# rasmusab/bayes.js

Hardware: AMD Instinct MI355X
Metric: posterior draws/sec (= param-updates/sec) (higher is better)
Workload: dtype f64

## Files before the change

### bayes.js_amd/csrc/amwg_kernel.h

```cpp
#pragma once
#if !defined(__HIPCC_RTC__)
#include <hip/hip_runtime.h>
#endif

#include "amwg_div.h"
#include "amwg_ld.h"
#include "amwg_philox.h"
#include "amwg_types.h"

namespace amwg {

struct LdsLayout {
  uint32_t data, state, pls, cnt, tot, cc, adapt, pl, idx, perm, total, stride, logpls, bc, xw;
};
__host__ __device__ inline LdsLayout lds_layout(size_t data_bytes, int P, int CPB, int max_top, int n_named, bool multi = false) {
  LdsLayout L;
  uint32_t o = 0;
  L.stride = (uint32_t)P | 1u;
  L.data = o;  o += (uint32_t)((data_bytes + 15) & ~(size_t)15);
  L.state = o; o += L.stride * CPB * 8;
  L.pls = o;   o += L.stride * CPB * 8;
  L.cnt = o;   o += L.stride * CPB * 8;
  L.tot = o;   o += (L.stride * CPB * 4 + 15) & ~15u;
  L.cc = o;    o += (uint32_t)P * sizeof(CompConst);
  L.adapt = o; o += ((uint32_t)P + 7) & ~7u;
  L.pl = o;    o += (uint32_t)n_named * 20u;
  o = (o + 15) & ~15u;
  L.idx = o;   o += (max_top > 1) ? (((uint32_t)max_top * CPB * (max_top > kByteTop ? 2u : 1u) + 15) & ~15u) : 0;
  L.perm = o;  o += (n_named > kPackedNamed) ? (((uint32_t)n_named * CPB * 2u + 15) & ~15u) : 0;
  L.logpls = o; o += multi ? L.stride * CPB * 8 : 0;
  L.bc = o;     o += multi ? ((L.stride * CPB * 4 + 15) & ~15u) : 0;
  L.xw = o;     o += multi ? 2u * 16u * 8u : 0;
  L.total = (o + 15) & ~15u;
  return L;
}

template <class Model, bool FAST, int G, int U = Model::kUnroll>
__device__ __forceinline__ double pass_over_data(const typename Model::Pass &ps, int n_obs, int sub, double acc) {
  const int n_full = n_obs / G, rem = n_obs % G;
  int k = 0;
  for (; k + U <= n_full; k += U) {
    double t[U];
#pragma unroll
    for (int u = 0; u < U; ++u) t[u] = Model::template term<FAST>(ps, (k + u) * G + sub);
#pragma unroll
    for (int u = 0; u < U; ++u) acc += t[u];
  }
  for (; k < n_full; ++k) acc += Model::template term<FAST>(ps, k * G + sub);
  if (sub < rem) acc += Model::template term<FAST>(ps, n_full * G + sub);
  return acc;
}

struct CrossWave {
  double *buf;
  int parity;
};

template <class...> using void_of = void;

template <class M, class = void> struct BinaryOf { static constexpr bool value = true; };
template <class M> struct BinaryOf<M, void_of<decltype(M::kHasBinary)>> { static constexpr bool value = M::kHasBinary; };

template <class M, class = void> struct TracksState { static constexpr bool value = false; };
template <class M> struct TracksState<M, void_of<decltype(M::kTracksState)>> { static constexpr bool value = M::kTracksState; };

template <class M, class = void> struct LaneReuseOf { static constexpr bool value = false; };
template <class M> struct LaneReuseOf<M, void_of<decltype(M::kLaneReuse)>> { static constexpr bool value = M::kLaneReuse; };

template <class M, class = void> struct CertifiedOf { static constexpr bool value = false; static constexpr int lanes = 0; };
template <class M> struct CertifiedOf<M, void_of<decltype(M::kCertified)>> { static constexpr bool value = M::kCertified; static constexpr int lanes = M::kCertifiedLanes; };
template <class M, int G, class = void> struct CertifiedAt { static constexpr bool value = false; };
template <class M, int G> struct CertifiedAt<M, G, void_of<decltype(M::kCertified)>> { static constexpr bool value = M::kCertified && M::kCertifiedLanes == G; };

template <class M, class = void> struct CertNeedsRows { static constexpr bool value = false; };
template <class M> struct CertNeedsRows<M, void_of<decltype(M::kCertifiedNeedsRows)>> { static constexpr bool value = M::kCertifiedNeedsRows; };

template <class M, class = void> struct RefOrderOf { static constexpr bool value = false; };
template <class M> struct RefOrderOf<M, void_of<decltype(M::kReferenceOrder)>> { static constexpr bool value = M::kReferenceOrder; };

template <class M, class = void> struct OwnPassOf { static constexpr bool value = false; };
template <class M> struct OwnPassOf<M, void_of<decltype(M::kOwnPass)>> { static constexpr bool value = M::kOwnPass; };

struct NoCache {};
template <class M, class = void> struct CacheOf { using type = NoCache; static __device__ __forceinline__ type init() { return type{}; } };
template <class M> struct CacheOf<M, void_of<typename M::Cache>> { using type = typename M::Cache; static __device__ __forceinline__ type init() { return M::cache_init(); } };

template <int OFF, bool EXACT = false>
__device__ __forceinline__ double xor_partner(double v) {
#if defined(__HIP_DEVICE_COMPILE__)
  int lo = (int)(uint32_t)f64_bits(v), hi = (int)(uint32_t)(f64_bits(v) >> 32);
  if constexpr (OFF == 1) {
    lo = __builtin_amdgcn_mov_dpp(lo, 0xB1, 0xF, 0xF, true); hi = __builtin_amdgcn_mov_dpp(hi, 0xB1, 0xF, 0xF, true);
  } else if constexpr (OFF == 2) {
    lo = __builtin_amdgcn_mov_dpp(lo, 0x4E, 0xF, 0xF, true); hi = __builtin_amdgcn_mov_dpp(hi, 0x4E, 0xF, 0xF, true);
  } else if constexpr (OFF == 4) {
    lo = __builtin_amdgcn_mov_dpp(lo, 0x141, 0xF, 0xF, true); hi = __builtin_amdgcn_mov_dpp(hi, 0x141, 0xF, 0xF, true);
    if constexpr (EXACT) {
      lo = __builtin_amdgcn_mov_dpp(lo, 0x1B, 0xF, 0xF, true); hi = __builtin_amdgcn_mov_dpp(hi, 0x1B, 0xF, 0xF, true);
    }
  } else if constexpr (OFF == 8) {
    lo = __builtin_amdgcn_mov_dpp(lo, 0x140, 0xF, 0xF, true); hi = __builtin_amdgcn_mov_dpp(hi, 0x140, 0xF, 0xF, true);
    if constexpr (EXACT) {
      lo = __builtin_amdgcn_mov_dpp(lo, 0x141, 0xF, 0xF, true); hi = __builtin_amdgcn_mov_dpp(hi, 0x141, 0xF, 0xF, true);
    }
  } else if constexpr (OFF == 16) {
    lo = __builtin_amdgcn_ds_swizzle(lo, 0x401F); hi = __builtin_amdgcn_ds_swizzle(hi, 0x401F);
  } else {
    return __shfl_xor(v, OFF, 64);
  }
  return bits_f64(((uint64_t)(uint32_t)hi << 32) | (uint64_t)(uint32_t)lo);
#else
  return v;
#endif
}
template <int OFF, bool EXACT = false>
__device__ __forceinline__ double xor_sum(double acc) {
#if defined(__HIP_DEVICE_COMPILE__)
  if constexpr (OFF == 16 || OFF == 32) {
    const uint32_t lo = (uint32_t)f64_bits(acc), hi = (uint32_t)(f64_bits(acc) >> 32);
    if constexpr (OFF == 32) {
      const auto l = __builtin_amdgcn_permlane32_swap(lo, lo, false, false), h = __builtin_amdgcn_permlane32_swap(hi, hi, false, false);
      return bits_f64(((uint64_t)h[0] << 32) | (uint64_t)l[0]) + bits_f64(((uint64_t)h[1] << 32) | (uint64_t)l[1]);
    } else {
      const auto l = __builtin_amdgcn_permlane16_swap(lo, lo, false, false), h = __builtin_amdgcn_permlane16_swap(hi, hi, false, false);
      return bits_f64(((uint64_t)h[0] << 32) | (uint64_t)l[0]) + bits_f64(((uint64_t)h[1] << 32) | (uint64_t)l[1]);
    }
  } else {
    return acc + xor_partner<OFF, EXACT>(acc);
  }
#else
  return acc;
#endif
}
template <int OFF, int LIMIT>
__device__ __forceinline__ double butterfly(double acc) {
  if constexpr (OFF < LIMIT) { acc = xor_sum<OFF>(acc); return butterfly<OFF * 2, LIMIT>(acc); }
  else return acc;
}

#ifndef AMWG_STEPPER_PRIORITY
#define AMWG_STEPPER_PRIORITY 2
#endif
constexpr int kStepperPriority = AMWG_STEPPER_PRIORITY;
__device__ __forceinline__ void wave_priority(int p) {
#if defined(__HIP_DEVICE_COMPILE__)
  if (kStepperPriority > 0) { if (p == 0) __builtin_amdgcn_s_setprio(0); else __builtin_amdgcn_s_setprio(kStepperPriority); }
#endif
}

__device__ __forceinline__ int fresh_uniform(int v) {
#if defined(__HIP_DEVICE_COMPILE__)
#if !defined(AMWG_X_NOFRESH)
  v = __builtin_amdgcn_readfirstlane(v);
  asm volatile("" : "+s"(v));
#endif
#endif
  return v;
}

template <class Model, int G, int U = 8>
__device__ __forceinline__ double log_post(const StateView &S, const StepArgs &a0, const unsigned char *smem, int sub, CrossWave &xw,
                                           typename CacheOf<Model>::type &cache) {
  struct { const ModelConsts &mc; DataRef d; } a{a0.mc, a0.d};
  a.d.n_obs = fresh_uniform(a0.d.n_obs);
  a.d.G = fresh_uniform(a0.d.G);
  double acc;
  if constexpr (Model::kUser) {
    wave_priority(0);
    bool summed = false;
    if constexpr (LaneReuseOf<Model>::value && G == 64) {
      if (a0.d.pad > 0) { acc = Model::template rows_eval<U>(cache, S, a.d, smem, sub, a0.d.pad, (int)(threadIdx.x >> 6)); summed = true; }
    }
    if (!summed) acc = Model::template eval<G, false>(S, a.d, smem, sub, nullptr);
  } else {
    if constexpr (TracksState<Model>::value) Model::template load<G>(cache, S, a.mc, a.d, smem, sub);
    const typename Model::Pass ps = Model::template begin<G>(S, a.mc, a.d, smem, cache);
    const double prior = Model::prior(S, a.mc, a.d, cache);
    acc = (sub == 0) ? prior : 0.0;
    if constexpr (Model::kSplitPrior) acc = Model::template prior_split<G>(S, a.mc, a.d, sub, acc, cache);
    wave_priority(0);
    bool summed = false;
    if constexpr (LaneReuseOf<Model>::value && G == 64) {
      if (ps.rows) { acc = Model::template lane_sum_rows<U>(cache, ps, acc, a.d.n_obs, a.d.G, sub, smem, a0.d.pad, (int)(threadIdx.x >> 6)); summed = true; }
    }
    if (summed) {
    } else if constexpr (Model::kHasFast) {
      if (ps.fast) acc = Model::template pass_fast<G, U>(ps, a.d.n_obs, sub, acc);
      else acc = Model::template pass_slow<G>(ps, a.d.n_obs, sub, acc);
    } else if constexpr (Model::kOneLanePass && G == 1) {
      acc = Model::pass_one_lane(ps, a.d.n_obs, acc);
    } else if constexpr (OwnPassOf<Model>::value) {
      acc = Model::template pass<G>(ps, a.d.n_obs, sub, acc);
    } else {
      acc = pass_over_data<Model, false, G>(ps, a.d.n_obs, sub, acc);
    }
    if constexpr (Model::kOneLanePass) {
      if (ps.has_invalid) acc = acc + (-kInf);
    }
  }
  wave_priority(kStepperPriority);
  acc = butterfly<1, (G < 64 ? G : 64)>(acc);
  if constexpr (G > 64) {
    constexpr int WV = G / 64;
    double *slot = xw.buf + xw.parity * 16;
    xw.parity ^= 1;
    const int wave = sub >> 6;
    if ((sub & 63) == 0) slot[wave] = acc;
    __syncthreads();
    double t[WV];
#pragma unroll
    for (int w = 0; w < WV; ++w) t[w] = slot[w];
#pragma unroll
    for (int off = 1; off < WV; off <<= 1) {
      double u[WV];
#pragma unroll
      for (int w = 0; w < WV; ++w) u[w] = t[w] + t[w ^ off];
#pragma unroll
      for (int w = 0; w < WV; ++w) t[w] = u[w];
    }
    acc = t[0];
  }
  return acc;
}

template <int G>
struct CoopStream {
  static constexpr int L = G < 64 ? G : 64;
  static constexpr int kLanesPerChain = G;
  uint32_t k0, k1, c2, c3;
  uint64_t b0;
  uint32_t pos;
  double u0, u1;
  int lane_in_chain, base_lane;
  static __device__ __attribute__((noinline)) Philox4 block(uint64_t b, uint32_t c2, uint32_t c3, uint32_t k0, uint32_t k1) {
    return philox4x32_10((uint32_t)b, (uint32_t)(b >> 32), c2, c3, k0, k1);
  }
  __device__ __forceinline__ void set_block(const Philox4 &w) { u0 = u53(w.w0, w.w1); u1 = u53(w.w2, w.w3); }
  __device__ __forceinline__ void fill() { set_block(block(b0 + (uint64_t)lane_in_chain, c2, c3, k0, k1)); }
  __device__ __forceinline__ void init(uint64_t seed, uint64_t chain, uint64_t consumed, int tid) {
    k0 = (uint32_t)seed; k1 = (uint32_t)(seed >> 32);
    c2 = (uint32_t)chain; c3 = (uint32_t)(chain >> 32);
    lane_in_chain = tid & (L - 1);
    base_lane = (tid & 63) & ~(L - 1);
    b0 = consumed >> 1;
    pos = (uint32_t)(consumed & 1u);
    fill();
  }
  __device__ __forceinline__ uint64_t consumed() const { return 2 * b0 + (uint64_t)pos; }
  __device__ __forceinline__ double next() {
    if constexpr (L == 64) {
      uint32_t p = (uint32_t)__builtin_amdgcn_readfirstlane((int)pos);
      if (p >= 128u) { b0 += 64ull; p = 0u; fill(); }
      const double mine = (p & 1u) ? u1 : u0;
      const int src = (int)(p >> 1);
      const uint32_t hi = (uint32_t)__builtin_amdgcn_readlane((int)(f64_bits(mine) >> 32), src);
      const uint32_t lo = (uint32_t)__builtin_amdgcn_readlane((int)(uint32_t)f64_bits(mine), src);
      pos = p + 1u;
      return bits_f64(((uint64_t)hi << 32) | (uint64_t)lo);
    } else {
      if (pos >= 2u * (uint32_t)L) { b0 += (uint64_t)L; pos = 0u; fill(); }
      double mine = (pos & 1u) ? u1 : u0;
      if constexpr (L > 1) mine = __shfl(mine, base_lane + (int)(pos >> 1), 64);
      ++pos;
      return mine;
    }
  }
};

template <int G>
__device__ __forceinline__ bool chain_true(bool c) {
#if defined(__HIP_DEVICE_COMPILE__)
  if constexpr (G >= 64) return __ballot(c) != 0ull;
#endif
  return c;
}

__device__ inline __attribute__((noinline)) int certified_test_wide(double dA, double eta, double u) {
  const double lo = dA - eta, hi = dA + eta;
  if (hi < -746.0) return -1;
  if (lo >= 0.0) return 1;
  if (!(eta < 0x1p+9) || !(u > 0x1p-60)) return 0;
  if (exp_v8(lo) * (1.0 - 0x1p-50) > u) return 1;
  if (exp_v8(hi) * (1.0 + 0x1p-50) < u) return -1;
  return 0;
}
__device__ __forceinline__ int certified_test(double dA, double eta, double ex, double u) {
  if (eta < 0x1p-7) return (ex * (1.0 - eta) > u && (u > 0.0 || dA > -700.0)) ? 1 : (ex * (1.0 + eta) < u ? -1 : 0);
  return certified_test_wide(dA, eta, u);
}

template <class Rng>
__device__ __forceinline__ double rnorm_js(Rng &rng, double mean, double sd) {
  constexpr int GU = Rng::kLanesPerChain;
  double u, v, q;
  bool again;
  do {
    u = rng.next();
    v = 1.7156 * (rng.next() - 0.5);
    const double x = u - 0.449871;
    const double y = __builtin_fabs(v) + 0.386595;
    q = x * x + y * (0.19600 * y - 0.25472 * x);
    again = false;
    if (chain_true<GU>(q > 0.27597)) again = chain_true<GU>(q > 0.27846) || chain_true<GU>(v * v > -4 * log_v8_cold(u) * u * u);
  } while (again);
  return (v / u) * sd + mean;
}

struct IndexColumn {
  unsigned char *base;
  int CPB;
  bool wide;
  __device__ __forceinline__ int get(int t) const {
    return wide ? (int)reinterpret_cast<const uint16_t *>(base)[t * CPB] : (int)base[t * CPB];
  }
  __device__ __forceinline__ void set(int t, int v) const {
    if (wide) reinterpret_cast<uint16_t *>(base)[t * CPB] = (uint16_t)v; else base[t * CPB] = (uint8_t)v;
  }
};
__device__ __forceinline__ uint32_t perm_get(uint64_t perm, int i) { return (uint32_t)(perm >> (4 * i)) & 0xFu; }
__device__ __forceinline__ uint64_t perm_swap(uint64_t perm, int i, int j) {
  const uint64_t d = ((perm >> (4 * i)) ^ (perm >> (4 * j))) & 0xFull;
  return perm ^ (d << (4 * i)) ^ (d << (4 * j));
}

__device__ __forceinline__ double js_max2(double a, double b) {
  if (a != a || b != b) return __builtin_nan("");
  if (a == b) return (a == 0 && __builtin_signbit(a)) ? b : a;
  return a > b ? a : b;
}

template <class M, int G, bool GL, bool SW = false> struct RngOf { using type = CoopStream<G>; };
template <class M, int G> struct RngOf<M, G, true, false> { using type = typename M::Stream; };
template <class M, int G> struct RngOf<M, G, false, true> { using type = typename M::SweepStream; };
template <class M, class = void> struct DynamicLdsOf { static constexpr bool value = false; };
template <class M> struct DynamicLdsOf<M, void_of<decltype(M::kDynamicLds)>> { static constexpr bool value = M::kDynamicLds; };
template <class M, bool GL> struct DataBytesOf {
  static __device__ __forceinline__ size_t get(const DataRef &d, int lanes, int threads) {
    if constexpr (DynamicLdsOf<M>::value) return M::lds_bytes_of(d, lanes, threads);
    else return M::lds_bytes(d.n_obs, d.G, lanes);
  }
};
template <class M> struct DataBytesOf<M, true> { static __device__ __forceinline__ size_t get(const DataRef &d, int, int threads) { return M::gl_lds_bytes(d.pad, threads / 64); } };

#if defined(__HIP_DEVICE_COMPILE__)
typedef const StepArgs __attribute__((address_space(4))) *cold_args_ptr;
__device__ __forceinline__ cold_args_ptr cold_args() {
  cold_args_ptr p = (cold_args_ptr)__builtin_amdgcn_kernarg_segment_ptr();
  asm volatile("" : "+s"(p));
  return p;
}
#else
typedef const StepArgs *cold_args_ptr;
__device__ inline cold_args_ptr cold_args() { return nullptr; }
#endif

struct SlotPre {
  int comp;
  double cur, sd, batch_size;
  int2 cnt;
  bool adapting;
};

__device__ __forceinline__ uint64_t uniform_u64(uint64_t v) {
#if defined(__HIP_DEVICE_COMPILE__)
  return ((uint64_t)(uint32_t)__builtin_amdgcn_readfirstlane((int)(uint32_t)(v >> 32)) << 32) | (uint64_t)(uint32_t)__builtin_amdgcn_readfirstlane((int)(uint32_t)v);
#else
  return v;
#endif
}
__device__ __forceinline__ int write_lane(int v, int value, int lane) {
#if defined(__HIP_DEVICE_COMPILE__)
  int keep;
  asm volatile("s_mov_b32 %1, m0\n\ts_mov_b32 m0, %3\n\tv_writelane_b32 %0, %2, m0\n\ts_mov_b32 m0, %1" : "+v"(v), "=&s"(keep) : "s"(value), "s"(lane));
#endif
  return v;
}

__device__ __forceinline__ void gl_resolve_unbounded(uint64_t EA, uint64_t OA, uint64_t EB, uint64_t OB, uint32_t &p, int &t, int top, int &ppv) {
#if defined(__HIP_DEVICE_COMPILE__)
  uint64_t m, rest;
  uint32_t tmp, keep_m0;
  asm volatile(
      "s_mov_b32 %[km0], m0\n"
      "1:\n\t"
      "s_cmp_ge_i32 %[t], %[top]\n\t"
      "s_cbranch_scc1 9f\n"
      "2:\n\t"
      "s_cmp_ge_u32 %[p], 0x100\n\t"
      "s_cbranch_scc1 9f\n\t"
      "s_bitcmp1_b32 %[p], 7\n\t"
      "s_cbranch_scc1 3f\n\t"
      "s_bitcmp1_b32 %[p], 0\n\t"
      "s_cselect_b64 %[m], %[OA], %[EA]\n\t"
      "s_branch 4f\n"
      "3:\n\t"
      "s_bitcmp1_b32 %[p], 0\n\t"
      "s_cselect_b64 %[m], %[OB], %[EB]\n"
      "4:\n\t"
      "s_bfe_u32 %[tmp], %[p], 0x60001\n\t"
      "s_lshr_b64 %[rest], %[m], %[tmp]\n\t"
      "s_cmp_lg_u64 %[rest], 0\n\t"
      "s_cbranch_scc1 6f\n\t"
      "s_and_b32 %[tmp], %[p], 1\n\t"
      "s_bitcmp1_b32 %[p], 7\n\t"
      "s_cbranch_scc1 5f\n\t"
      "s_or_b32 %[p], %[tmp], 0x80\n\t"
      "s_branch 2b\n"
      "5:\n\t"
      "s_or_b32 %[p], %[tmp], 0xfe\n\t"
      "s_branch 9f\n"
      "6:\n\t"
      "s_ff1_i32_b64 %[tmp], %[rest]\n\t"
      "s_lshl_b32 %[tmp], %[tmp], 1\n\t"
      "s_add_u32 %[p], %[p], %[tmp]\n\t"
      "s_mov_b32 m0, %[t]\n\t"
      "v_writelane_b32 %[ppv], %[p], m0\n\t"
      "s_add_u32 %[p], %[p], 3\n\t"
      "s_add_u32 %[t], %[t], 1\n\t"
      "s_branch 1b\n"
      "9:\n\t"
      "s_mov_b32 m0, %[km0]"
      : [p] "+s"(p), [t] "+s"(t), [ppv] "+v"(ppv), [m] "=&s"(m), [rest] "=&s"(rest), [tmp] "=&s"(tmp), [km0] "=&s"(keep_m0)
      : [EA] "s"(EA), [OA] "s"(OA), [EB] "s"(EB), [OB] "s"(OB), [top] "s"(top)
      : "scc");
#endif
}

template <int G>
__device__ __forceinline__ int chain_uniform(int v) {
#if defined(__HIP_DEVICE_COMPILE__)
  if constexpr (G >= 64) return __builtin_amdgcn_readfirstlane(v);
#endif
  return v;
}

__device__ __forceinline__ double lane_value(double v, int src) {
#if defined(__HIP_DEVICE_COMPILE__)
  const uint32_t hi = (uint32_t)__builtin_amdgcn_readlane((int)(f64_bits(v) >> 32), src);
  const uint32_t lo = (uint32_t)__builtin_amdgcn_readlane((int)(uint32_t)f64_bits(v), src);
  return bits_f64(((uint64_t)hi << 32) | (uint64_t)lo);
#else
  return v;
#endif
}

constexpr int kErrReplicasNeedOneWave = 1, kErrLaunchTooLong = 2, kErrMirrorOutOfSync = 4, kErrSweepNeedsOrderInRegisters = 8, kErrNoKernelBody = 16;
__device__ __forceinline__ void device_error(const StepArgs &a, int code) {
#if defined(__HIP_DEVICE_COMPILE__)
  if (threadIdx.x == 0) (void)atomicOr(a.ch.error, code);
#endif
}
template <class M, class = void> struct MirrorCheckOf { static constexpr bool value = false; };
template <class M> struct MirrorCheckOf<M, void_of<decltype(M::kMirrorCheck)>> { static constexpr bool value = M::kMirrorCheck; };

template <class Model, int G, int BT = 256, bool GL = false, bool SW = false, bool CT = false>
__device__ __forceinline__ void step_body(const StepArgs &a, unsigned char *smem) {
  constexpr int kPassU = SW ? (CertNeedsRows<Model>::value ? 2 : 4) : (BT >= 1024 ? 4 : 8);
  const int tid = threadIdx.x, nt = blockDim.x;
  constexpr bool kMulti = G > 64;
  if (!kMulti && a.cpb > 0 && nt != 64) { device_error(a, kErrReplicasNeedOneWave); return; }
  if (a.n_steps > 65535) { device_error(a, kErrLaunchTooLong); return; }
  const int CPB = kMulti ? G / 64 : ((a.cpb > 0 && a.cpb < nt / G) ? a.cpb : nt / G);
  const int c_raw = kMulti ? tid / 64 : tid / G;
  const int c_in = c_raw < CPB ? c_raw : CPB - 1, sub = tid % G;
  const int P = a.pl.P;
  const int n_named = a.pl.n_params;
  const LdsLayout L = lds_layout(DataBytesOf<Model, GL>::get(a.d, G, nt), P, CPB, a.pl.max_top, n_named, kMulti);

  const unsigned char *data_lds = smem + L.data;
  double *Sblk = reinterpret_cast<double *>(smem + L.state);
  CompConst *cc = reinterpret_cast<CompConst *>(smem + L.cc);
  uint8_t *adapt = smem + L.adapt;
  int32_t *pl_base = reinterpret_cast<int32_t *>(smem + L.pl), *pl_len = pl_base + n_named, *pl_top = pl_len + n_named, *pl_multidim = pl_top + n_named, *pl_inner = pl_multidim + n_named;
  const bool wide_idx = a.pl.max_top > kByteTop, wide_perm = n_named > kPackedNamed;
  const IndexColumn idx{smem + L.idx + (wide_idx ? 2 * c_in : c_in), CPB, wide_idx};
  const IndexColumn pcol{smem + L.perm + 2 * c_in, CPB, true};
  double *SDme = reinterpret_cast<double *>(smem + L.pls) + (size_t)c_in * L.stride;
  int2 *CNTme = reinterpret_cast<int2 *>(smem + L.cnt) + (size_t)c_in * L.stride;
  uint32_t *TOTme = reinterpret_cast<uint32_t *>(smem + L.tot) + (size_t)c_in * L.stride;
  double *LOGPLSme = reinterpret_cast<double *>(smem + L.logpls) + (size_t)c_in * L.stride;
  int32_t *BCme = reinterpret_cast<int32_t *>(smem + L.bc) + (size_t)c_in * L.stride;
  CrossWave xw{reinterpret_cast<double *>(smem + L.xw), 0};
  typename CacheOf<Model>::type cache = CacheOf<Model>::init();

  Model::stage(smem + L.data, a.d, tid, nt, G);
  for (int p = tid; p < P; p += nt) { cc[p] = a.cc[p]; adapt[p] = a.is_adapting[p]; }
  for (int i = tid; i < 4 * n_named; i += nt) pl_base[i] = a.pl.tab[i];
  for (int i = tid; i < n_named; i += nt) pl_inner[i] = a.pl.tab[n_named + i] / a.pl.tab[2 * n_named + i];

  const int64_t chain_raw = kMulti ? (int64_t)blockIdx.x : (int64_t)blockIdx.x * CPB + c_in;
  const bool live = chain_raw < a.C;
  const int64_t cl = live ? chain_raw : a.C - 1;
  const bool writer = live && sub == 0;
  const bool counter = sub == 0 && c_raw < CPB;
  const int64_t C = a.C;

  double *Sme = Sblk + (size_t)c_in * L.stride;
  for (int p = 0; p < P; ++p) {
    Sme[p] = a.ch.state[p * C + cl];
    SDme[p] = exp_v8(a.ch.prop_log_scale[p * C + cl]);
    CNTme[p] = make_int2(a.ch.acceptance_count[p * C + cl], a.ch.iterations_since_adaption[p * C + cl]);
    TOTme[p] = 0u;
    if constexpr (kMulti) { LOGPLSme[p] = a.ch.prop_log_scale[p * C + cl]; BCme[p] = a.ch.batch_count[p * C + cl]; }
  }
  const StateView S{Sme};
  uint64_t perm = wide_perm ? 0ull : a.ch.perm[cl];
  if (wide_perm)
    for (int k = 0; k < n_named; ++k) pcol.set(k, (int)a.ch.perm16[(int64_t)k * C + cl]);
  typename RngOf<Model, G, GL, SW>::type rng;
  if constexpr (GL) rng.init(a.seed, a.chain_offset + (uint64_t)cl, a.ch.rng_n[cl], tid, reinterpret_cast<double *>(smem + L.data + Model::gl_lds_bytes(a.d.pad, 0)) + (size_t)(tid >> 6) * 256);
  else if constexpr (SW) rng.init(a.seed, a.chain_offset + (uint64_t)cl, a.ch.rng_n[cl], tid, reinterpret_cast<double *>(smem + L.data + Model::window_offset(a.d, nt / 64)) + (size_t)(tid >> 6) * 256);
  else rng.init(a.seed, a.chain_offset + (uint64_t)cl, a.ch.rng_n[cl], tid);
  double lp_curr = a.ch.lp_curr[cl];
  __syncthreads();
  constexpr bool kCert = CT && CertifiedAt<Model, G>::value && !GL && (SW == CertNeedsRows<Model>::value);
  static_assert(kCert == CT, "a certified kernel is instantiated for a model that has no certified value at this lane count");
  constexpr bool kRefOrder = kCert && G > 1 && RefOrderOf<Model>::value;
  auto expression = [&]() -> double {
    if constexpr (kRefOrder) return Model::template reference_order<G>(cache, S, a.mc, a.d, data_lds, sub);
    else if constexpr (!GL) return log_post<Model, G, kPassU>(S, a, data_lds, sub, xw, cache);
    else return 0.0;
  };
  if constexpr (!GL) { if (a.init_lp) lp_curr = expression(); }
  double lpA = lp_curr, epsA = 0.0;
  bool lp_exact = true;
  if constexpr (kCert) { if (!a.init_lp) { epsA = a.ch.lp_eps[cl]; lp_exact = epsA == 0.0; } }
  (void)lpA; (void)epsA; (void)lp_exact;
#if defined(AMWG_AUDIT)
  constexpr bool kAudit = kCert;
#else
  constexpr bool kAudit = false;
#endif
  [[maybe_unused]] double audE = 0.0, aud_max_v = 0.0, aud_max_d = 0.0;
  [[maybe_unused]] uint32_t aud_n = 0u, aud_bad = 0u;
  [[maybe_unused]] auto audit_bin = [&](int which, double ratio) {
#if defined(AMWG_AUDIT)
    if (writer) {
      int b = 0;
      if (ratio > 0.0) { b = (int)((f64_bits(ratio) >> 52) & 0x7ffu) - 1023 + 40; b = b < 1 ? 1 : (b > 63 ? 63 : b); }
      if (!(ratio == ratio)) b = 63;
      (void)atomicAdd(cold_args()->ch.audit_hist + which * 64 + b, 1ull);
    }
#endif
  };
  [[maybe_unused]] auto audit_adversarial_u = [&](double ex, double eta, double u, int parity) -> double {
    if (!(eta < 0x1p-8) || !(ex > 0x1p-900) || !(ex < kInf)) return u;
    const double below = ex * (1.0 - 1.5 * eta), above = ex * (1.0 + 1.5 * eta);
    const double v = ((parity & 1) && above < 1.0) ? above : below;
    return (v > 0.0 && v < 1.0) ? v : u;
  };
  [[maybe_unused]] auto audit_value = [&](double A, double eps, double E) {
    if (eps == eps && eps < kInf && eps > 0.0 && E == E && __builtin_fabs(E) < kInf) {
      const double r = __builtin_fabs(A - E) / eps;
      aud_max_v = (r > aud_max_v || !(r == r)) ? r : aud_max_v;
      audit_bin(0, r);
    }
  };
  [[maybe_unused]] auto audit_difference = [&](double dA, double eta0, double dE, int verdict, double u) {
    if (eta0 == eta0 && eta0 < kInf && eta0 > 0.0 && dE == dE && __builtin_fabs(dE) < kInf) {
      const double r = __builtin_fabs(dA - dE) / eta0;
      aud_max_d = (r > aud_max_d || !(r == r)) ? r : aud_max_d;
      audit_bin(1, r);
    }
    const bool exact_acc = exp_v8(dE) > u;
    ++aud_n;
    if ((verdict > 0 && !exact_acc) || (verdict < 0 && exact_acc)) ++aud_bad;
  };
#if defined(AMWG_X_PHASES)
  uint64_t ph_acc[16];
#pragma unroll
  for (int q = 0; q < 16; ++q) ph_acc[q] = 0;
  uint64_t ph_last = __builtin_readcyclecounter();
#define AMWG_PHASE(i) do { const uint64_t ph_now = __builtin_readcyclecounter(); ph_acc[i] += ph_now - ph_last; ph_last = ph_now; } while (0)
#else
#define AMWG_PHASE(i) do { } while (0)
#endif
  auto set_state = [&](int comp, double v) {
    Sme[comp] = v;
    if constexpr (TracksState<Model>::value) Model::on_set(cache, comp, v, sub, a.d);
  };

  constexpr int D = Model::kDerived;
  const int PR = P + D;
  int64_t row = a.row0;
  int32_t next_rec = (int32_t)a.step0;
  const int P_stepped = a.pl.P_stepped;
  const bool recording = a.draws != nullptr;
  const int n_steps = a.n_steps;

  const int lane64 = tid & 63;
  int ord = lane64;
  (void)ord;
  if (SW && a.pl.max_top > 64) { device_error(a, kErrSweepNeedsOrderInRegisters); return; }
  const bool ord_in_regs = SW ? true : (G >= 64 && a.pl.max_top <= 64);
  constexpr bool kSweep = SW && !GL && LaneReuseOf<Model>::value && G == 64 && !BinaryOf<Model>::value;
  const bool sweep_rt = kSweep && ord_in_regs && a.d.pad > 0;
  if constexpr (kAudit) { if (lp_exact) audE = lp_curr; else audE = expression(); }
  wave_priority(kStepperPriority);
  auto record_draws = [&](int step) {
    if (recording && step == next_rec) {
      double *const draws = cold_args()->draws;
// ... 680 lines not shown
```

### bayes.js_amd/csrc/amwg_pass.h

```cpp
#pragma once
#include "amwg_div.h"
#include "amwg_types.h"

namespace amwg {

#if defined(__HIP_DEVICE_COMPILE__)
#define AMWG_STAGE_FENCE() __builtin_amdgcn_sched_barrier(0)
#else
#define AMWG_STAGE_FENCE() ((void)0)
#endif

template <int U>
struct NormBlock { double v[U]; };

#if defined(__HIP_DEVICE_COMPILE__)
#define AMWG_WAIT_LDS_LE(n) __builtin_amdgcn_s_waitcnt(0xC07F | ((n) << 8))
#else
#define AMWG_WAIT_LDS_LE(n) ((void)0)
#endif

template <int U, bool ADD_PREV>
AMWG_HD void norm_block_stages(NormBlock<U> &b, const double (&m)[U], NormBlock<U> &q, const NormBlock<U> &prev, double &acc,
                                                  double c, double den, Reciprocal y) {
  int a = 0;
// ... 43 lines not shown
    const XT *px = x + sub;
    const uint8_t *pg = g + sub;
    auto load_idx = [&](int blk, int (&gi)[U]) {
      if constexpr (GATHER) {
        blk = blk < n_blocks ? blk : n_blocks - 1;
#pragma unroll
        for (int u = 0; u < U; ++u) gi[u] = pg[(blk * U + u) * G];
      }
    };
    auto load_val = [&](int blk, NormBlock<U> &xv, double (&mv)[U], const int (&gi)[U]) {
#pragma unroll
      for (int u = 0; u < U; ++u) xv.v[u] = (double)px[(blk * U + u) * G];
#pragma unroll
      for (int u = 0; u < U; ++u) mv[u] = GATHER ? S(gi[u]) : mean;
    };
    load_idx(0, ga);
    load_val(0, xa, ma, ga);
    load_idx(1, gb);
    AMWG_STAGE_FENCE();
    if (n_blocks > 1) { load_val(1, xb, mb, gb); load_idx(2, ga); }
    AMWG_STAGE_FENCE();
    norm_block_stages<U, false>(xa, ma, qa, qa, acc, c, den, y);
    int blk = 1;
    for (; blk + 2 < n_blocks; blk += 2) {
      load_val(blk + 1, xa, ma, ga);
      load_idx(blk + 2, gb);
      AMWG_STAGE_FENCE();
      if constexpr (!GATHER && U == 8 && sizeof(XT) == 8) { AMWG_WAIT_LDS_LE(4); AMWG_STAGE_FENCE(); }
      norm_block_stages<U, true>(xb, mb, qb, qa, acc, c, den, y);
      load_val(blk + 2, xb, mb, gb);
      load_idx(blk + 3, ga);
      AMWG_STAGE_FENCE();
      if constexpr (!GATHER && U == 8 && sizeof(XT) == 8) { AMWG_WAIT_LDS_LE(4); AMWG_STAGE_FENCE(); }
      norm_block_stages<U, true>(xa, ma, qa, qb, acc, c, den, y);
    }
    if (blk < n_blocks) {
      if (blk + 1 < n_blocks) load_val(blk + 1, xa, ma, ga);
      AMWG_STAGE_FENCE();
      norm_block_stages<U, true>(xb, mb, qb, qa, acc, c, den, y);
      if (blk + 1 < n_blocks) {
        norm_block_stages<U, true>(xa, ma, qa, qb, acc, c, den, y);
#pragma unroll
        for (int u = 0; u < U; ++u) acc = acc + qa.v[u];
      } else {
#pragma unroll
        for (int u = 0; u < U; ++u) acc = acc + qb.v[u];
      }
    } else {
#pragma unroll
      for (int u = 0; u < U; ++u) acc = acc + qa.v[u];
    }
    k = n_blocks * U;
  }
  const int left = n_full - k;
  if (left + (rem > 0 ? 1 : 0) <= U / 2 + 1) {
    constexpr int TMAX = U / 2 + 1;
    double xv[TMAX], mv[TMAX];
    const int cnt_all = left + (rem > 0 ? 1 : 0);
    if (cnt_all > 0) {
#pragma unroll
    for (int r = 0; r < TMAX; ++r) {
      int i = (k + (r < cnt_all ? r : 0)) * G + sub;
      i = i < n_obs ? i : n_obs - 1;
      xv[r] = (double)x[i];
      mv[r] = GATHER ? S(g[i]) : mean;
    }
    AMWG_STAGE_FENCE();
#pragma unroll
    for (int r = 0; r < TMAX; ++r) {
      if (r < cnt_all) {
        const double t = xv[r] - mv[r];
        const double term = c - div_by_invariant(t * t, den, y);
        const bool mine = r < left || sub < rem;
        acc = mine ? acc + term : acc;
      }
    }
    }
  } else if (left > 0 || rem > 0) {
    const int cnt = left + (sub < rem ? 1 : 0);
    NormBlock<U> xt, qt;
    double mt[U];
#pragma unroll
    for (int u = 0; u < U; ++u) {
      int r = u < cnt ? u : (cnt > 0 ? cnt - 1 : 0);
      int i = (k + r) * G + sub;
      i = i < n_obs ? i : n_obs - 1;
      xt.v[u] = (double)x[i];
      mt[u] = GATHER ? S(g[i]) : mean;
    }
    AMWG_STAGE_FENCE();
    norm_block_stages<U, false>(xt, mt, qt, qt, acc, c, den, y);
#pragma unroll
    for (int u = 0; u < U; ++u) acc = u < cnt ? acc + qt.v[u] : acc;
  }
  return acc;
}

#if defined(__HIP_DEVICE_COMPILE__)
typedef const double __attribute__((address_space(4))) *amwg_uniform_f64_ptr;
#else
typedef const double *amwg_uniform_f64_ptr;
#endif

struct StagedFirst { static constexpr bool value = true; };
struct StagedLater { static constexpr bool value = false; };

template <int U>
AMWG_HD double norm_pass_uniform(const double *x_global, double mean, double c, double den, Reciprocal y, int n_obs, double acc) {
  constexpr int CH = 2 * U;
  const int n_chunks = n_obs / CH;
  int k = 0;
  if (n_chunks > 0) {
    amwg_uniform_f64_ptr px = (amwg_uniform_f64_ptr)(uintptr_t)x_global;
    double ma[U];
#pragma unroll
    for (int u = 0; u < U; ++u) ma[u] = mean;
    NormBlock<CH> sa, sb;
    NormBlock<U> ta, tb, qa, qb;
    auto load_chunk = [&](int ch, NormBlock<CH> &dst) {
      ch = ch < n_chunks ? ch : n_chunks - 1;
#pragma unroll
      for (int u = 0; u < CH; ++u) dst.v[u] = px[ch * CH + u];
    };
    auto lo = [&](const NormBlock<CH> &src, NormBlock<U> &t) {
#pragma unroll
      for (int u = 0; u < U; ++u) t.v[u] = src.v[u];
    };
    auto hi = [&](const NormBlock<CH> &src, NormBlock<U> &t) {
#pragma unroll
      for (int u = 0; u < U; ++u) t.v[u] = src.v[U + u];
    };
    auto compute = [&](const NormBlock<CH> &src, auto first) {
      lo(src, ta);
      norm_block_stages<U, !decltype(first)::value>(ta, ma, qa, qb, acc, c, den, y);
      hi(src, tb);
      norm_block_stages<U, true>(tb, ma, qb, qa, acc, c, den, y);
    };
    load_chunk(0, sb);
    AMWG_WAIT_LDS_LE(0); AMWG_STAGE_FENCE();
    load_chunk(1, sa);
    AMWG_STAGE_FENCE();
    compute(sb, StagedFirst{});
    int ch = 1;
    for (; ch + 1 < n_chunks; ch += 2) {
      AMWG_WAIT_LDS_LE(0); AMWG_STAGE_FENCE();
      load_chunk(ch + 1, sb);
      AMWG_STAGE_FENCE();
      compute(sa, StagedLater{});
      AMWG_WAIT_LDS_LE(0); AMWG_STAGE_FENCE();
      load_chunk(ch + 2, sa);
      AMWG_STAGE_FENCE();
      compute(sb, StagedLater{});
    }
    if (ch < n_chunks) {
      AMWG_WAIT_LDS_LE(0); AMWG_STAGE_FENCE();
      compute(sa, StagedLater{});
    }
#pragma unroll
    for (int u = 0; u < U; ++u) acc = acc + qb.v[u];
    k = n_chunks * CH;
  }
  for (; k < n_obs; ++k) {
    const double t = x_global[k] - mean;
    acc += c - div_by_invariant(t * t, den, y);
  }
  return acc;
}

template <int U>
AMWG_HD double norm_sq_pass_uniform(const double *x_global, double mean, int n_obs) {
  constexpr int CH = 2 * U;
  double acc[U];
#pragma unroll
  for (int u = 0; u < U; ++u) acc[u] = 0.0;
  const int n_chunks = n_obs / CH;
  int k = 0;
  if (n_chunks > 0) {
    amwg_uniform_f64_ptr px = (amwg_uniform_f64_ptr)(uintptr_t)x_global;
    NormBlock<CH> sa, sb;
    auto load_chunk = [&](int ch, NormBlock<CH> &dst) {
      ch = ch < n_chunks ? ch : n_chunks - 1;
#pragma unroll
      for (int u = 0; u < CH; ++u) dst.v[u] = px[ch * CH + u];
    };
    auto compute = [&](const NormBlock<CH> &src) {
#pragma unroll
      for (int u = 0; u < U; ++u) { const double t = src.v[u] - mean; acc[u] = __builtin_fma(t, t, acc[u]); }
      AMWG_STAGE_FENCE();
#pragma unroll
      for (int u = 0; u < U; ++u) { const double t = src.v[U + u] - mean; acc[u] = __builtin_fma(t, t, acc[u]); }
      AMWG_STAGE_FENCE();
    };
    load_chunk(0, sb);
    AMWG_WAIT_LDS_LE(0); AMWG_STAGE_FENCE();
    load_chunk(1, sa);
    AMWG_STAGE_FENCE();
    compute(sb);
    int ch = 1;
    for (; ch + 1 < n_chunks; ch += 2) {
      AMWG_WAIT_LDS_LE(0); AMWG_STAGE_FENCE();
      load_chunk(ch + 1, sb);
      AMWG_STAGE_FENCE();
      compute(sa);
      AMWG_WAIT_LDS_LE(0); AMWG_STAGE_FENCE();
      load_chunk(ch + 2, sa);
      AMWG_STAGE_FENCE();
      compute(sb);
    }
    if (ch < n_chunks) {
      AMWG_WAIT_LDS_LE(0); AMWG_STAGE_FENCE();
      compute(sa);
    }
    k = n_chunks * CH;
  }
  for (; k < n_obs; ++k) {
    const double t = x_global[k] - mean;
    acc[0] = __builtin_fma(t, t, acc[0]);
  }
  double s = 0.0;
#pragma unroll
  for (int u = 0; u < U; ++u) s += acc[u];
  return s;
}

struct PassRows { int blocks, full, masked; };
AMWG_HD PassRows pass_rows(int n_obs, int B) { const int rows = n_obs / 64; return PassRows{rows / B, rows % B, (n_obs % 64) != 0 ? 1 : 0}; }
AMWG_HD constexpr int pass_part_slot(int B, int p) { return B - 2 * p; }
AMWG_HD constexpr int pass_part_row(int full, int p) { return full & ~(2 * p - 1); }
#if defined(__HIPCC__) || defined(__HIPCC_RTC__)
#ifndef AMWG_WAVE_BLOCK
#define AMWG_WAVE_BLOCK 16
#endif
constexpr int kWaveBlock = AMWG_WAVE_BLOCK;
template <int N> struct PassBlock { static constexpr int value = N; };
typedef int amwg_v16i __attribute__((ext_vector_type(16)));
__device__ __forceinline__ double *wave_scratch_of(const DataRef &d) {
#if defined(__HIP_DEVICE_COMPILE__)
  if (!d.wave_scratch) return nullptr;
  const uint32_t wave = (uint32_t)__builtin_amdgcn_readfirstlane((int)(blockIdx.x * (blockDim.x >> 6) + (threadIdx.x >> 6)));
  return d.wave_scratch + (size_t)wave * 64;
#else
  (void)d; return nullptr;
#endif
}
#if defined(__HIP_DEVICE_COMPILE__)
typedef const double __attribute__((address_space(3))) *amwg_lds_f64_ptr;
#else
typedef const double *amwg_lds_f64_ptr;
#endif
template <int B, bool SCALAR_ONLY = false, class XP = const double *>
__device__ __forceinline__ double norm_sq_pass_wave(XP x, double mu, int n_obs, double *scr = nullptr) {
#if defined(__HIP_DEVICE_COMPILE__)
  int lane = (int)(threadIdx.x & 63u);
  asm volatile("" : "+v"(lane));
  double a[64];
#pragma unroll
  for (int c = 0; c < 64; ++c) a[c] = 0.0;
  const int mu_lo = (int)(uint32_t)f64_bits(mu), mu_hi = (int)(uint32_t)(f64_bits(mu) >> 32);
  auto mean_of = [&](int c) { return bits_f64(((uint64_t)(uint32_t)__builtin_amdgcn_readlane(mu_hi, c) << 32) | (uint64_t)(uint32_t)__builtin_amdgcn_readlane(mu_lo, c)); };
  bool smem_done = false;
#if !defined(AMWG_X_NO_SMEM_MEANS)
  if (SCALAR_ONLY || scr != nullptr) {
    const PassRows pr = pass_rows(n_obs, B);
    double xv[B];
    auto read_rows = [&](int blk, int b0, int b1) {
#pragma unroll
      for (int b = b0; b < b1; ++b) xv[b] = x[(blk * B + b) * 64 + lane];
    };
    if (pr.blocks > 0) read_rows(0, 0, B);
    scr[lane] = mu;
    asm volatile("s_waitcnt vmcnt(0)\n\ts_dcache_inv\n\ts_waitcnt lgkmcnt(0)" ::: "memory");
    auto fetch = [&](int g) { amwg_v16i r; asm volatile("s_load_dwordx16 %0, %1, %2" : "=&s"(r) : "s"(scr), "s"(g * 8)); return r; };
    auto landed = [&](amwg_v16i &r) { asm volatile("s_waitcnt lgkmcnt(0)" : "+s"(r)); };
    auto mean_in = [&](const amwg_v16i &r, int j) { return bits_f64(((uint64_t)(uint32_t)r[2 * j + 1] << 32) | (uint64_t)(uint32_t)r[2 * j]); };
    amwg_v16i cur = fetch(0);
    landed(cur);
    auto rows_s = [&](auto r0, auto rn, auto refill) {
      constexpr int R0 = decltype(r0)::value, RN = decltype(rn)::value, RH = R0 + RN / 2;
#pragma unroll
      for (int g = 0; g < 64; g += 8) {
        amwg_v16i nxt = fetch(g + 8 < 64 ? g + 8 : 0);
        AMWG_STAGE_FENCE();
#pragma unroll
        for (int b = R0; b < RH; ++b) {
#pragma unroll
          for (int j = 0; j < 8; ++j) { const double t = xv[b] - mean_in(cur, j); a[g + j] = __builtin_fma(t, t, a[g + j]); }
        }
        if (g + 8 == 64) { AMWG_STAGE_FENCE(); refill(R0, RH); AMWG_STAGE_FENCE(); }
#pragma unroll
        for (int b = RH; b < R0 + RN; ++b) {
#pragma unroll
          for (int j = 0; j < 8; ++j) { const double t = xv[b] - mean_in(cur, j); a[g + j] = __builtin_fma(t, t, a[g + j]); }
        }
        if (g + 8 == 64) AMWG_STAGE_FENCE();
        landed(nxt);
        if (g + 8 == 64) { AMWG_STAGE_FENCE(); refill(RH, R0 + RN); AMWG_STAGE_FENCE(); }
        cur = nxt;
      }
    };
    for (int k = 0; k < pr.blocks; ++k) {
      const int nb = k + 1 < pr.blocks ? k + 1 : k;
      rows_s(PassBlock<0>{}, PassBlock<B>{}, [&](int b0, int b1) { read_rows(nb, b0, b1); });
    }
    if (pr.full > 0 || pr.masked) {
      const int rbase = pr.blocks * B * 64 + lane;
      const bool has = pr.masked && rbase + pr.full * 64 < n_obs;
      auto read_part = [&](auto pt) {
        constexpr int P = decltype(pt)::value;
        if (pr.full & P) {
#pragma unroll
          for (int b = 0; b < P; ++b) xv[pass_part_slot(B, P) + b] = x[rbase + (pass_part_row(pr.full, P) + b) * 64];
        }
      };
      if constexpr (B >= 32) read_part(PassBlock<16>{});
      if constexpr (B >= 16) read_part(PassBlock<8>{});
      if constexpr (B >= 8) read_part(PassBlock<4>{});
      if constexpr (B >= 4) read_part(PassBlock<2>{});
      if constexpr (B >= 2) read_part(PassBlock<1>{});
      if (pr.masked) xv[B - 1] = x[has ? rbase + pr.full * 64 : 0];
      auto part = [&](auto pt) {
        constexpr int P = decltype(pt)::value;
        if (pr.full & P) rows_s(PassBlock<pass_part_slot(B, P)>{}, pt, [](int, int) {});
      };
      if constexpr (B >= 32) part(PassBlock<16>{});
      if constexpr (B >= 16) part(PassBlock<8>{});
      if constexpr (B >= 8) part(PassBlock<4>{});
      if constexpr (B >= 4) part(PassBlock<2>{});
      if constexpr (B >= 2) part(PassBlock<1>{});
      if (pr.masked) {
        const double xm = xv[B - 1];
#pragma unroll
        for (int g = 0; g < 64; g += 8) {
          amwg_v16i nxt = cur;
          if (g + 8 < 64) nxt = fetch(g + 8);
#pragma unroll
          for (int j = 0; j < 8; ++j) { const double t = has ? xm - mean_in(cur, j) : 0.0; a[g + j] = __builtin_fma(t, t, a[g + j]); }
          if (g + 8 < 64) landed(nxt);
          cur = nxt;
        }
      }
    }
    smem_done = true;
  }
#endif
  if constexpr (!SCALAR_ONLY) if (!smem_done) {
  auto block = [&](auto tag, int at) {
    constexpr int BB = decltype(tag)::value;
    double xv[BB];
#pragma unroll
    for (int b = 0; b < BB; ++b) xv[b] = x[at + b * 64 + lane];
#pragma unroll
    for (int g = 0; g < 64; g += 8) {
      double m[8];
#pragma unroll
      for (int j = 0; j < 8; ++j) m[j] = mean_of(g + j);
#pragma unroll
      for (int b = 0; b < BB; ++b) {
#pragma unroll
        for (int j = 0; j < 8; ++j) { const double t = xv[b] - m[j]; a[g + j] = __builtin_fma(t, t, a[g + j]); }
      }
    }
  };
  int base = 0;
  for (; base + 64 * B <= n_obs; base += 64 * B) block(PassBlock<B>{}, base);
  if constexpr (B >= 32) { if (base + 64 * 16 <= n_obs) { block(PassBlock<16>{}, base); base += 64 * 16; } }
  if constexpr (B >= 16) { if (base + 64 * 8 <= n_obs) { block(PassBlock<8>{}, base); base += 64 * 8; } }
  if constexpr (B >= 8) { if (base + 64 * 4 <= n_obs) { block(PassBlock<4>{}, base); base += 64 * 4; } }
  if constexpr (B >= 4) { if (base + 64 * 2 <= n_obs) { block(PassBlock<2>{}, base); base += 64 * 2; } }
  if constexpr (B >= 2) { if (base + 64 <= n_obs) { block(PassBlock<1>{}, base); base += 64; } }
  for (; base + 64 <= n_obs; base += 64) block(PassBlock<1>{}, base);
  if (base < n_obs) {
    const int i = base + lane;
    const bool has = i < n_obs;
    const double xv = x[has ? i : base];
#pragma unroll
    for (int g = 0; g < 64; g += 8) {
      double m[8];
#pragma unroll
      for (int j = 0; j < 8; ++j) m[j] = mean_of(g + j);
#pragma unroll
      for (int j = 0; j < 8; ++j) { const double t = has ? xv - m[j] : 0.0; a[g + j] = __builtin_fma(t, t, a[g + j]); }
    }
  }
  }
  auto swap_add = [&](double A, double Bv, int off) {
    const uint32_t al = (uint32_t)f64_bits(A), ah = (uint32_t)(f64_bits(A) >> 32), bl = (uint32_t)f64_bits(Bv), bh = (uint32_t)(f64_bits(Bv) >> 32);
    if (off == 32) {
      const auto l = __builtin_amdgcn_permlane32_swap(al, bl, false, false), h = __builtin_amdgcn_permlane32_swap(ah, bh, false, false);
      return bits_f64(((uint64_t)h[0] << 32) | (uint64_t)l[0]) + bits_f64(((uint64_t)h[1] << 32) | (uint64_t)l[1]);
    } else {
      const auto l = __builtin_amdgcn_permlane16_swap(al, bl, false, false), h = __builtin_amdgcn_permlane16_swap(ah, bh, false, false);
      return bits_f64(((uint64_t)h[0] << 32) | (uint64_t)l[0]) + bits_f64(((uint64_t)h[1] << 32) | (uint64_t)l[1]);
    }
  };
#pragma unroll
  for (int j = 0; j < 32; ++j) a[j] = swap_add(a[j], a[j + 32], 32);
#pragma unroll
  for (int j = 0; j < 16; ++j) a[j] = swap_add(a[j], a[j + 16], 16);
  {
    const bool up = (lane & 8) != 0;
#pragma unroll
    for (int j = 0; j < 8; ++j) { const double send = up ? a[j] : a[j + 8], keep = up ? a[j + 8] : a[j]; a[j] = keep + xor_partner<8, true>(send); }
  }
  {
    const bool up = (lane & 4) != 0;
#pragma unroll
    for (int j = 0; j < 4; ++j) { const double send = up ? a[j] : a[j + 4], keep = up ? a[j + 4] : a[j]; a[j] = keep + xor_partner<4, true>(send); }
  }
  {
    const bool up = (lane & 2) != 0;
#pragma unroll
    for (int j = 0; j < 2; ++j) { const double send = up ? a[j] : a[j + 2], keep = up ? a[j + 2] : a[j]; a[j] = keep + xor_partner<2>(send); }
  }
  {
    const bool up = (lane & 1) != 0;
    const double send = up ? a[0] : a[1], keep = up ? a[1] : a[0];
    a[0] = keep + xor_partner<1>(send);
  }
  return a[0];
#else
  (void)x; (void)mu; (void)n_obs;
  return 0.0;
#endif
}
#endif

}
```

### bayes.js_amd/csrc/amwg_philox.h

```cpp
#pragma once
#include "amwg_math.h"

namespace amwg {

struct Philox4 { uint32_t w0, w1, w2, w3; };

AMWG_HD uint32_t mulhi32(uint32_t a, uint32_t b) {
#if defined(__HIP_DEVICE_COMPILE__)
  return __umulhi(a, b);
#else
  return (uint32_t)(((uint64_t)a * b) >> 32);
#endif
}

AMWG_HD Philox4 philox4x32_10(uint32_t c0, uint32_t c1, uint32_t c2, uint32_t c3, uint32_t k0, uint32_t k1) {
#pragma unroll
  for (int r = 0; r < 10; ++r) {
    const uint64_t p0 = (uint64_t)0xD2511F53u * c0, p1 = (uint64_t)0xCD9E8D57u * c2;
    const uint32_t hi0 = (uint32_t)(p0 >> 32), lo0 = (uint32_t)p0;
    const uint32_t hi1 = (uint32_t)(p1 >> 32), lo1 = (uint32_t)p1;
    c0 = hi1 ^ c1 ^ k0;
    c2 = hi0 ^ c3 ^ k1;
    c1 = lo1;
    c3 = lo0;
    k0 += 0x9E3779B9u;
    k1 += 0xBB67AE85u;
  }
  return Philox4{c0, c1, c2, c3};
}

AMWG_HD double u53(uint32_t hi, uint32_t lo) {
  return (double)(((uint64_t)hi << 21) | (uint64_t)(lo >> 11)) * 1.1102230246251565e-16;
}

struct ChainStream {
  uint32_t k0, k1, c2, c3;
  uint64_t n;
  uint32_t r2, r3;

  AMWG_HD void init(uint64_t seed, uint64_t chain, uint64_t consumed) {
    k0 = (uint32_t)seed; k1 = (uint32_t)(seed >> 32);
    c2 = (uint32_t)chain; c3 = (uint32_t)(chain >> 32);
    n = consumed;
    r2 = r3 = 0;
    if (n & 1) {
      const uint64_t b = n >> 1;
      const Philox4 w = philox4x32_10((uint32_t)b, (uint32_t)(b >> 32), c2, c3, k0, k1);
      r2 = w.w2; r3 = w.w3;
    }
  }
  AMWG_HD double next() {
    double u;
    if ((n & 1) == 0) {
      const uint64_t b = n >> 1;
      const Philox4 w = philox4x32_10((uint32_t)b, (uint32_t)(b >> 32), c2, c3, k0, k1);
      r2 = w.w2; r3 = w.w3;
      u = u53(w.w0, w.w1);
    } else {
      u = u53(r2, r3);
    }
    ++n;
    return u;
  }
};

}
```

Before: 1.424 billion.

## Draw normal proposal uniforms in pairs and move ragged-tail rows after reduction

Adds a paired-uniform draw for the single-lane RNG stream so each Box-Muller-like ratio-of-uniforms attempt takes both uniforms from one Philox fill instead of two separate next() calls. In the sum-of-squares pass, the masked remainder rows (n_obs not a multiple of 64) are no longer processed as a full 64-mean wide block. Instead they are loaded once, broadcast via readlane, and accumulated per lane after the cross-lane reduction, since each lane handles its own chain mean mu. This removes a whole padded 64x64 FMA sweep for the tail, at the cost of a serial loop over up to 63 leftover rows per lane.

```diff
diff --git a/bayes.js_amd/csrc/amwg_kernel.h b/bayes.js_amd/csrc/amwg_kernel.h
--- a/bayes.js_amd/csrc/amwg_kernel.h
+++ b/bayes.js_amd/csrc/amwg_kernel.h
@@ -265,6 +265,10 @@
       return mine;
     }
   }
+  __device__ __forceinline__ void next_pair(double &a, double &b) {
+    static_assert(L == 1, "the pair draw is the one-lane stream's");
+    stream_next_pair(*this, a, b);
+  }
 };
 
 template <int G>
@@ -295,8 +299,10 @@
   double u, v, q;
   bool again;
   do {
-    u = rng.next();
-    v = 1.7156 * (rng.next() - 0.5);
+    double r;
+    if constexpr (GU == 1) rng.next_pair(u, r);
+    else { u = rng.next(); r = rng.next(); }
+    v = 1.7156 * (r - 0.5);
     const double x = u - 0.449871;
     const double y = __builtin_fabs(v) + 0.386595;
     q = x * x + y * (0.19600 * y - 0.25472 * x);
diff --git a/bayes.js_amd/csrc/amwg_pass.h b/bayes.js_amd/csrc/amwg_pass.h
--- a/bayes.js_amd/csrc/amwg_pass.h
+++ b/bayes.js_amd/csrc/amwg_pass.h
@@ -369,9 +369,8 @@
       const int nb = k + 1 < pr.blocks ? k + 1 : k;
       rows_s(PassBlock<0>{}, PassBlock<B>{}, [&](int b0, int b1) { read_rows(nb, b0, b1); });
     }
-    if (pr.full > 0 || pr.masked) {
+    if (pr.full > 0) {
       const int rbase = pr.blocks * B * 64 + lane;
-      const bool has = pr.masked && rbase + pr.full * 64 < n_obs;
       auto read_part = [&](auto pt) {
         constexpr int P = decltype(pt)::value;
         if (pr.full & P) {
@@ -384,7 +383,6 @@
       if constexpr (B >= 8) read_part(PassBlock<4>{});
       if constexpr (B >= 4) read_part(PassBlock<2>{});
       if constexpr (B >= 2) read_part(PassBlock<1>{});
-      if (pr.masked) xv[B - 1] = x[has ? rbase + pr.full * 64 : 0];
       auto part = [&](auto pt) {
         constexpr int P = decltype(pt)::value;
         if (pr.full & P) rows_s(PassBlock<pass_part_slot(B, P)>{}, pt, [](int, int) {});
@@ -394,18 +392,6 @@
       if constexpr (B >= 8) part(PassBlock<4>{});
       if constexpr (B >= 4) part(PassBlock<2>{});
       if constexpr (B >= 2) part(PassBlock<1>{});
-      if (pr.masked) {
-        const double xm = xv[B - 1];
-#pragma unroll
-        for (int g = 0; g < 64; g += 8) {
-          amwg_v16i nxt = cur;
-          if (g + 8 < 64) nxt = fetch(g + 8);
-#pragma unroll
-          for (int j = 0; j < 8; ++j) { const double t = has ? xm - mean_in(cur, j) : 0.0; a[g + j] = __builtin_fma(t, t, a[g + j]); }
-          if (g + 8 < 64) landed(nxt);
-          cur = nxt;
-        }
-      }
     }
     smem_done = true;
   }
@@ -436,20 +422,10 @@
   if constexpr (B >= 4) { if (base + 64 * 2 <= n_obs) { block(PassBlock<2>{}, base); base += 64 * 2; } }
   if constexpr (B >= 2) { if (base + 64 <= n_obs) { block(PassBlock<1>{}, base); base += 64; } }
   for (; base + 64 <= n_obs; base += 64) block(PassBlock<1>{}, base);
-  if (base < n_obs) {
-    const int i = base + lane;
-    const bool has = i < n_obs;
-    const double xv = x[has ? i : base];
-#pragma unroll
-    for (int g = 0; g < 64; g += 8) {
-      double m[8];
-#pragma unroll
-      for (int j = 0; j < 8; ++j) m[j] = mean_of(g + j);
-#pragma unroll
-      for (int j = 0; j < 8; ++j) { const double t = has ? xv - m[j] : 0.0; a[g + j] = __builtin_fma(t, t, a[g + j]); }
-    }
-  }
-  }
+  }
+  const int rem = __builtin_amdgcn_readfirstlane(n_obs & 63);
+  double xl = 0.0;
+  if (rem != 0) xl = x[n_obs - rem + (lane < rem ? lane : 0)];
   auto swap_add = [&](double A, double Bv, int off) {
     const uint32_t al = (uint32_t)f64_bits(A), ah = (uint32_t)(f64_bits(A) >> 32), bl = (uint32_t)f64_bits(Bv), bh = (uint32_t)(f64_bits(Bv) >> 32);
     if (off == 32) {
@@ -484,7 +460,29 @@
     const double send = up ? a[0] : a[1], keep = up ? a[1] : a[0];
     a[0] = keep + xor_partner<1>(send);
   }
-  return a[0];
+  double s = a[0];
+  if (rem != 0) {
+    const int xl_lo = (int)(uint32_t)f64_bits(xl), xl_hi = (int)(uint32_t)(f64_bits(xl) >> 32);
+    auto leftover = [&](int k) { return bits_f64(((uint64_t)(uint32_t)__builtin_amdgcn_readlane(xl_hi, k) << 32) | (uint64_t)(uint32_t)__builtin_amdgcn_readlane(xl_lo, k)); };
+    int k = 0;
+    for (; k + 8 <= rem; k += 8) {
+      double t[8];
+#pragma unroll
+      for (int j = 0; j < 8; ++j) t[j] = leftover(k + j) - mu;
+      AMWG_STAGE_FENCE();
+      double e = t[1] * t[1];
+      s = __builtin_fma(t[0], t[0], s);
+#pragma unroll
+      for (int j = 2; j < 8; j += 2) { e = __builtin_fma(t[j + 1], t[j + 1], e); s = __builtin_fma(t[j], t[j], s); }
+      s = s + e;
+    }
+#pragma unroll 1
+    for (; k < rem; ++k) {
+      const double t = leftover(k) - mu;
+      s = __builtin_fma(t, t, s);
+    }
+  }
+  return s;
 #else
   (void)x; (void)mu; (void)n_obs;
   return 0.0;
diff --git a/bayes.js_amd/csrc/amwg_philox.h b/bayes.js_amd/csrc/amwg_philox.h
--- a/bayes.js_amd/csrc/amwg_philox.h
+++ b/bayes.js_amd/csrc/amwg_philox.h
@@ -64,4 +64,14 @@
   }
 };
 
+template <class S>
+AMWG_HD void stream_next_pair(S &s, double &a, double &b) {
+  const uint32_t p = s.pos;
+  const double held = s.u1;
+  if (p != 0u) { s.b0 += 1; s.fill(); }
+  a = p == 1u ? held : s.u0;
+  b = p == 1u ? s.u0 : s.u1;
+  s.pos = p == 1u ? 1u : 2u;
 }
+
+}
```

Result: faster. 1.444 billion (median of 6 runs) (+1.4%).
